# agakshat/spacefortress

Hardware: AMD Instinct MI355X
Metric: env-steps/sec (whole node), youturn random-action rollout @65536 envs/GPU (higher is better)
Workload: dtype f64; 1 GPU; youturn, 65536 envs/GPU, features obs (f32), uniform random discrete actions resident in HBM, per-lane auto-reset; envs_per_gpu=65536, gametype=youturn, obs_type=features

## Files before the change

### spacefortress_amd/csrc/sf_kernels.hip

```cpp
#include <hip/hip_runtime.h>
#include <cstdio>
#include <cstdlib>
#include <stdint.h>

#include "sf_drawrec.h"
#include "sf_lane_dev.h"
#define SF_EVENTS_FN static __device__ __forceinline__
#include "sf_events.h"

#ifndef SF_BLOCK
#define SF_BLOCK 256
#endif
#ifndef SF_SPLIT
#define SF_SPLIT 1
#endif
#ifndef SF_MROWS
#define SF_MROWS 3
#endif
#ifndef SF_SPF
#define SF_SPF 6
#endif
#ifndef SF_STAGGER
#define SF_STAGGER 12
#endif
// ... 145 lines not shown
template <int DIM>
__device__ __forceinline__ void write_features_f32(float* o, const Lane& L, const Extras& e, int real_shell_count) {
  const int n_missiles = __popc(L.mmask);
  const int n_shells = real_shell_count ? __popc(L.smask) : n_missiles;
  const int kill_ready = (L.vlner > 10 && L.fort_vuln_t < sfc::vuln_time) ? 1 : 0;
  const int timers[4] = {L.fire_t, L.thrust_t, L.left_t, L.right_t};
  o[0] = (L.fl & SF_FL_SHIP_ALIVE) ? 1.0f : 0.0f;
  o[1] = (float)L.sx;
  o[2] = (float)L.sy;
  o[3] = (float)L.vx;
  o[4] = (float)L.vy;
  o[5] = (float)L.angle;
  o[6] = (float)e.aim;
  o[7] = (float)e.vdir;
  o[8] = (float)e.ndist;
  o[9] = (L.fl & SF_FL_FORT_ALIVE) ? 1.0f : 0.0f;
  o[10] = (float)L.fort_angle;
  o[11] = (float)L.vlner;
  o[12] = (float)kill_ready;
  o[13] = (float)n_missiles;
  o[14] = (float)n_shells;
#pragma unroll
  for (int k = 0; k < DIM - 15; k++) o[15 + k] = (float)timers[k];
}
template <int DIM>
__device__ __forceinline__ void flush_features_f32(const float* stage_w, float* dst_w, unsigned lane) {
  __builtin_amdgcn_fence(__ATOMIC_RELEASE, "wavefront");
  __builtin_amdgcn_wave_barrier();
  __builtin_amdgcn_fence(__ATOMIC_ACQUIRE, "wavefront");
  typedef float f4_t __attribute__((ext_vector_type(4)));
  constexpr int NV = 64 * DIM / 4, IT = (NV + 63) / 64;
  f4_t v[IT];
#pragma unroll
  for (int k = 0; k < IT; k++)
    if (k * 64 + 63 < NV || (int)lane + k * 64 < NV) v[k] = reinterpret_cast<const f4_t*>(stage_w)[lane + k * 64];
#pragma unroll
  for (int k = 0; k < IT; k++)
    if (k * 64 + 63 < NV || (int)lane + k * 64 < NV) {
      sf_store<f4_t>(reinterpret_cast<f4_t*>(dst_w) + lane + k * 64, v[k]);
    }
}

template <typename T>
__device__ __forceinline__ void flush_obs_wave(const SfKernelArgs& a, const T* stage_w, T* obs, unsigned wave_env0,
                                               unsigned lane, bool vec_ok) {
  __builtin_amdgcn_fence(__ATOMIC_RELEASE, "wavefront");
  __builtin_amdgcn_wave_barrier();
  __builtin_amdgcn_fence(__ATOMIC_ACQUIRE, "wavefront");
  long rows = (long)a.n_envs - (long)wave_env0;
  if (rows > 64) rows = 64;
  if (rows <= 0) return;
  const int total = (int)rows * a.obs_dim;
  T* dst = obs + (size_t)wave_env0 * a.obs_dim;
  constexpr int V = 16 / (int)sizeof(T);
  int done_elems = 0;
  if (vec_ok) {
    typedef T vec_t __attribute__((ext_vector_type(V)));
    const int nvec = total / V;
    for (int v = lane; v < nvec; v += 64) {
      sf_store<vec_t>(reinterpret_cast<vec_t*>(dst) + v, reinterpret_cast<const vec_t*>(stage_w)[v]);
    }
    done_elems = nvec * V;
  }
  for (int t = done_elems + lane; t < total; t += 64) dst[t] = stage_w[t];
}

template <typename T>
__device__ __forceinline__ void norm_partials_wave(const SfKernelArgs& a, T* stage_w, unsigned wave_env0, unsigned lane,
                                                   double my_ret, bool has_obs) {
  const int dim = a.obs_dim, groups = 64 / dim;
  const size_t waves = (size_t)(a.lanes / 64), w = wave_env0 >> 6;
  long rows = (long)a.n_envs - (long)wave_env0;
  rows = rows > 64 ? 64 : (rows < 0 ? 0 : rows);
  double s = 0, q = 0;
  if (has_obs && (int)lane < groups * dim)
    for (int r = (int)lane / dim; r < rows; r += groups) {
      const double v = (double)stage_w[r * dim + (int)lane % dim];
      s += v;
      q += v * v;
    }
  __builtin_amdgcn_wave_barrier();
  double* fold = reinterpret_cast<double*>(stage_w);
  if (has_obs) {
    fold[lane] = s;
    fold[64 + lane] = q;
  }
  __builtin_amdgcn_fence(__ATOMIC_RELEASE, "wavefront");
  __builtin_amdgcn_wave_barrier();
  __builtin_amdgcn_fence(__ATOMIC_ACQUIRE, "wavefront");
  if ((int)lane < dim) {
    double ts = 0, tq = 0;
    if (has_obs)
      for (int g = 0; g < groups; g++) {
        ts += fold[g * dim + lane];
        tq += fold[64 + g * dim + lane];
      }
    a.n_partials[(size_t)lane * waves + w] = ts;
    a.n_partials[(size_t)(dim + 1 + lane) * waves + w] = tq;
  }
  double rs = (long)lane < rows ? my_ret : 0.0, rq = rs * rs;
  for (int o = 32; o > 0; o >>= 1) {
    rs += __shfl_xor(rs, o);
    rq += __shfl_xor(rq, o);
  }
  if (lane == 0) {
    a.n_partials[(size_t)dim * waves + w] = rs;
    a.n_partials[(size_t)(2 * dim + 1) * waves + w] = rq;
  }
}

}

__global__ __launch_bounds__(SF_BLOCK) void sf_reset_kernel(SfKernelArgs a, int first, unsigned cursor0,
                                                           unsigned cursor_stride, void* obs) {
  const unsigned i = blockIdx.x * SF_BLOCK + threadIdx.x;
  const unsigned lane = threadIdx.x & 63u;
  unsigned char* const tb = a.state + (size_t)__builtin_amdgcn_readfirstlane(i >> 6) * sfl::kTileBytes;
  const Off o = {lane * 16u, lane * 8u, lane * 4u, lane * 2u, lane};
  Lane L;
  if (first) {
    L.prev_vlner = 0;
    L.cursor = cursor0 + cursor_stride * i;
  } else {
    const i4_t mi = SF_LD(i4_t, SF_CHUNK(misc, 0), o.o16);
    L.prev_vlner = SF_LD(int, SF_CHUNK(timers_a, 0), o.o16) & 0xFFF;
    L.cursor = (unsigned)mi.y;
  }
  new_game(a, L);
  L.mpool = 0;
  store_lane(tb, o, L);
  if (obs != nullptr && i < (unsigned)a.n_envs && a.obs_type != 3) {
    Extras e = compute_extras(a, L, sf_atan2<true>(L.sy - sfc::fort_y, L.sx - sfc::fort_x), sf_atan2<false>(L.vy, L.vx));
    if (a.ref_reset_obs) e = Extras{0.0, 0.0, 0.0};
    write_obs_row(a, obs, i, L, e);
  }
}

template <bool AUTOTURN, bool SHAPED, bool FUSED, int OBSK, bool XTRA, int BLKP, bool FOBS = false>
__global__ __launch_bounds__(BLKP > 2000 ? BLKP - 2000 : (BLKP > 1000 ? 2 * (BLKP - 1000) : BLKP)) void sf_step_kernel(unsigned char* state_p, const double* consts_p,
                                                          const void* actions, int n_envs_p, int act_type,
                                                          int32_t* reward_out, uint8_t* done_out, uint8_t* info_out,
                                                          SfKernelArgs a, void* obs, int obs_vec_ok, int n_steps) {
  constexpr bool REPEAT = BLKP > 2000;
  constexpr bool SPLIT = BLKP > 1000 && !REPEAT;
  constexpr int BLK = REPEAT ? BLKP - 2000 : (SPLIT ? BLKP - 1000 : BLKP);
  constexpr int NT = SPLIT ? 2 * BLK : BLK;
  static_assert(!SPLIT || (!FUSED && OBSK == 1 && !XTRA), "the split launch exists for the plain step of the default observation");
  static_assert(!FOBS || XTRA, "the final-observation output rides on the XTRA instantiations");
  static_assert(!REPEAT || (FUSED && XTRA && !FOBS && BLK == SF_BLOCK), "the action repeat rides on the fused XTRA instantiations (a.final_obs: a run-time test)");
  constexpr int kStaged = SPLIT ? SF_LDS_SPLIT_DOUBLES : SF_LDS_DOUBLES;
  constexpr int kTrigPieces = (kStaged / 2 + NT - 1) / NT;
  constexpr int kLdsEv = kStaged;
  constexpr int kLdsAtab = SPLIT ? SF_CONST_ATAB : kLdsEv + BLK, kLdsHand = SPLIT ? kLdsEv + BLK : kLdsAtab + SF_ATAB_DOUBLES,
                kLdsHandMeta = kLdsHand + 2 * BLK,
                kLdsHandFlags = kLdsHandMeta + BLK / 2, kLdsStage = SPLIT ? kLdsHandFlags + BLK / 32 : kLdsHand;
  static_assert(kLdsEv == SF_LDS_EV || SPLIT, "the other kernels' map is the one above");
  static_assert(kStaged % 2 == 0 && kLdsAtab % 2 == 0 && kLdsHand % 2 == 0 && kLdsStage % 2 == 0, "16-byte LDS accesses");
  extern __shared__ double lds[];
  const unsigned tid_all = threadIdx.x;
  const unsigned tid = SPLIT ? (tid_all & (unsigned)(BLK - 1)) : tid_all;
  const unsigned i = blockIdx.x * BLK + tid;
  const unsigned lane = tid & 63u;
  unsigned char* const tb = state_p + (size_t)__builtin_amdgcn_readfirstlane(i >> 6) * sfl::kTileBytes;
  const Off o = {lane * 16u, lane * 8u, lane * 4u, lane * 2u, lane};
  const Off g = {i * 16u, i * 8u, i * 4u, i * 2u, i};
  const bool real = i < (unsigned)n_envs_p;
  const __amdgpu_buffer_rsrc_t rs = __builtin_amdgcn_make_buffer_rsrc(tb, 0, (int)sfl::kTileBytes, 0x00020000);
  constexpr int kStAux = SF_SC_AUX;
  auto pld16 = [&](unsigned goff, bool p) __attribute__((always_inline)) -> d2_t {
    return __builtin_bit_cast(d2_t, __builtin_amdgcn_raw_buffer_load_b128(rs, p ? o.o16 : SF_OOB, goff, 0));
  };
  auto pst16 = [&](unsigned goff, bool p, d2_t v) __attribute__((always_inline)) {
    sf_buf_st128<kStAux>(__builtin_bit_cast(u4_t, v), rs, p ? o.o16 : SF_OOB, goff);
  };
  auto pst16_at = [&](unsigned goff, bool p, unsigned extra, d2_t v) __attribute__((always_inline)) {
    sf_buf_st128<kStAux>(__builtin_bit_cast(u4_t, v), rs, p ? o.o16 + extra : SF_OOB, goff);
  };
#ifdef SF_STAMPS
  unsigned long long stamp_[SF_STAMP_SLOTS] = {};
  stamp_[12] = __builtin_amdgcn_s_memrealtime();
#endif
  SF_STAMP(0, false);

#if SF_STAGGER
  if (n_envs_p > 65536 - 256 && ((blockIdx.x >> 3) & 1u)) __builtin_amdgcn_s_sleep(SF_STAGGER);
#endif
  constexpr unsigned kSpinLimit = 1u << 18;
  typedef volatile __attribute__((address_space(3))) unsigned lds_word_t;
  lds_word_t* const hflags = (lds_word_t*)(reinterpret_cast<unsigned*>(lds + kLdsHandFlags) + 4u * (tid >> 6));
  if constexpr (SPLIT) {
    if (tid_all >= (unsigned)BLK) {
      const unsigned n_word = *reinterpret_cast<const __attribute__((address_space(4))) unsigned*>(
          reinterpret_cast<const __attribute__((address_space(4))) void*>(
              (unsigned long long)(tb + (unsigned)sfl::chunk_offset(SF_G_misc, 0) + 8u)));
      unsigned cpi0[kTrigPieces];
      d2_t cst0[kTrigPieces];
#pragma unroll
      for (int k = 0; k < kTrigPieces; k++) {
        cpi0[k] = min(tid_all + k * NT, (unsigned)(kStaged / 2 - 1));
        cst0[k] = SF_LD(d2_t, (const unsigned char*)consts_p, cpi0[k] * 16u);
      }
      const unsigned m_live = n_word >> SF_MPOOL_SHIFT;
      d2_t prow[SF_MROWS];
      unsigned pmeta[SF_MROWS];
#pragma unroll
      for (int k = 0; k < kTrigPieces; k++) reinterpret_cast<d2_t*>(lds)[cpi0[k]] = cst0[k];
      if (lane < 4u) hflags[lane] = 0u;
      asm volatile("" ::: "memory");
#pragma unroll
      for (int r = 0; r < SF_MROWS; r++) {
        asm volatile("" : "=v"(prow[r].x), "=v"(prow[r].y));
        pmeta[r] = 0u;
        if (m_live > 64u * r) {
          const bool in_ = 64u * r + lane < m_live;
          prow[r] = __builtin_bit_cast(d2_t, __builtin_amdgcn_raw_buffer_load_b128(rs, in_ ? o.o16 : SF_OOB, SF_GOFF(missile_pos, r), 0));
          pmeta[r] = __builtin_amdgcn_raw_buffer_load_b32(rs, in_ ? o.o4 : SF_OOB, SF_GOFF(missile_meta, r), 0);
        }
      }
      __syncthreads();
#pragma unroll
      for (int r = 0; r < SF_MROWS; r++) asm volatile("" : "+v"(pmeta[r]));
      const double* trig = lds;
      d2_t pcs[SF_MROWS];
#pragma unroll
      for (int r = 0; r < SF_MROWS; r++) pcs[r] = *reinterpret_cast<const d2_t*>(&trig[2 * SF_MM_ANGLE(pmeta[r])]);
      double kv_speed = sfc::missile_speed, kv_fx = sfc::fort_x, kv_fy = sfc::fort_y, kv_w = sfc::width_d, kv_h = sfc::height_d,
             kv_mr2 = sfc::missile_hit_r2;
      asm volatile("" : "+v"(kv_speed), "+v"(kv_fx), "+v"(kv_fy), "+v"(kv_w), "+v"(kv_h), "+v"(kv_mr2));
      unsigned wp = 0;
      unsigned* const evw32 = reinterpret_cast<unsigned*>(lds + kLdsEv) + 2u * (tid & ~63u);
      auto m_row = [&](double x, double y, unsigned meta, d2_t cs, bool valid) __attribute__((always_inline)) {
        const double nx = x + kv_speed * cs.x, ny = y + kv_speed * cs.y;
        const double dx = nx - kv_fx, dy = ny - kv_fy;
        const bool hit = valid & (dx * dx + dy * dy <= kv_mr2);
        const bool gone = valid & (hit | (__builtin_fmax(__builtin_fmax(-nx, nx - kv_w), __builtin_fmax(-ny, ny - kv_h)) > 0));
        if (__ballot(gone) != 0ull) {
          if (gone)
            __hip_atomic_fetch_or(evw32 + 2 * SF_MM_OWNER(meta) + (hit ? 0 : 1), 1u << SF_MM_SLOT(meta), __ATOMIC_RELAXED,
                                  __HIP_MEMORY_SCOPE_WORKGROUP);
        }
        const bool keep = valid & !gone;
        const unsigned long long kb = __ballot(keep);
        const unsigned idx = wp + __builtin_amdgcn_mbcnt_hi((unsigned)(kb >> 32), __builtin_amdgcn_mbcnt_lo((unsigned)kb, 0u));
        wp += (unsigned)__popcll(kb);
        sf_buf_st128<kStAux>(__builtin_bit_cast(u4_t, (d2_t{nx, ny})), rs, keep ? idx * 16u : SF_OOB,
                                               SF_GOFF(missile_pos, 0));
        __builtin_amdgcn_raw_buffer_store_b32(meta, rs, keep ? idx * 4u : SF_OOB, SF_GOFF(missile_meta, 0), kStAux);
      };
#pragma unroll
      for (int r = 0; r < SF_MROWS; r++)
        if (m_live > 64u * r) m_row(prow[r].x, prow[r].y, pmeta[r], pcs[r], 64u * r + lane < m_live);
      if (m_live > 64u * SF_MROWS) {
#pragma unroll 1
        for (unsigned r = SF_MROWS; 64u * r < m_live; r++) {
          const d2_t pr = __builtin_bit_cast(d2_t, __builtin_amdgcn_raw_buffer_load_b128(rs, o.o16 + r * 1024u, SF_GOFF(missile_pos, 0), 16));
          const unsigned pm = __builtin_amdgcn_raw_buffer_load_b32(rs, o.o4 + r * 256u, SF_GOFF(missile_meta, 0), 16);
          m_row(pr.x, pr.y, pm, *reinterpret_cast<const d2_t*>(&trig[2 * SF_MM_ANGLE(pm)]), 64u * r + lane < m_live);
        }
      }
      unsigned fired, spins = 0u;
      while ((fired = (unsigned)__builtin_amdgcn_readfirstlane((int)hflags[0])) == 0u && ++spins < kSpinLimit) __builtin_amdgcn_s_sleep(1);
      if (spins >= kSpinLimit && lane == 0u) atomicAdd(&a.acc[SF_ACC_HANDOVER], 1ull);
      asm volatile("" ::: "memory");
      if (fired == 2u) {
        const d2_t nxy = reinterpret_cast<const d2_t*>(lds + kLdsHand)[tid];
        const unsigned nm = reinterpret_cast<const unsigned*>(lds + kLdsHandMeta)[tid];
        m_row(nxy.x, nxy.y, nm & 0x7FFFFFFFu, *reinterpret_cast<const d2_t*>(&trig[2 * SF_MM_ANGLE(nm)]), !(nm >> 31));
      }
      asm volatile("s_waitcnt lgkmcnt(0)" ::: "memory");
      if (lane == 0u) hflags[1] = 0x80000000u | wp;
      asm volatile("s_waitcnt vmcnt(0)" ::: "memory");
      if (lane == 0u) hflags[2] = 1u;
      return;
    }
  }
  u4_t act_rec = {0u, 0u, 0u, 0u};
  if (XTRA && act_type == SF_ACT_SAMPLED)
    act_rec = *(reinterpret_cast<const __attribute__((address_space(4))) u4_t*>(
                    reinterpret_cast<const __attribute__((address_space(4))) void*>((unsigned long long)actions)) +
                __builtin_amdgcn_readfirstlane(i >> 6));
  auto sample_action = [&](int step) __attribute__((always_inline)) -> int {
    const unsigned x = sf_philox4x32_10(act_rec.w + lane, act_rec.x + (unsigned)step, act_rec.y, act_rec.z);
    return real ? (int)__umulhi(x, (unsigned)a.n_actions) : 0;
  };
  auto load_action = [&](int step) __attribute__((always_inline)) -> int {
    if (!real || (XTRA && act_type == SF_ACT_SAMPLED)) return 0;
    const unsigned char* ab = (const unsigned char*)actions;
    const unsigned e = (unsigned)step * (unsigned)n_envs_p + i;
    if (act_type == 8) return (int)SF_LD(long long, ab, e * 8u);
    if (act_type == 4) return SF_LD(int, ab, e * 4u);
    return SF_LD(unsigned char, ab, e);
  };
  Lane L;
  load_lane_early(tb, o, L);
  int act_next = load_action(0);
  const unsigned atab_pi = min(tid, (unsigned)(SF_ATAB_DOUBLES / 2 - 1));
  const d2_t atab_piece = SPLIT ? d2_t{0, 0} : SF_LD(d2_t, (const unsigned char*)consts_p, (SF_CONST_ATAB / 2 + atab_pi) * 16u);
  const unsigned char* cb = (const unsigned char*)consts_p;
  d2_t cst[kTrigPieces];
  unsigned cpi[kTrigPieces];
#pragma unroll
  for (int k = 0; k < kTrigPieces; k++) {
    cpi[k] = min(tid_all + k * NT, (unsigned)(kStaged / 2 - 1));
    cst[k] = SF_LD(d2_t, cb, cpi[k] * 16u);
  }
  int act_sampled = 0;
  if (XTRA && act_type == SF_ACT_SAMPLED) act_sampled = sample_action(0);
#define SF_LOAD_POOL_ROWS(aux, n_pool)                                                                                        \
  _Pragma("unroll") for (int r = 0; r < SF_MROWS; r++) {                                                                      \
    const bool in_ = 64u * r + lane < (n_pool);                                                                               \
    prow[r] = __builtin_bit_cast(d2_t, __builtin_amdgcn_raw_buffer_load_b128(rs, in_ ? o.o16 : SF_OOB, SF_GOFF(missile_pos, r), (aux)));   \
    pmeta[r] = __builtin_amdgcn_raw_buffer_load_b32(rs, in_ ? o.o4 : SF_OOB, SF_GOFF(missile_meta, r), (aux));               \
  }
  constexpr bool kPoolLoads = !SPLIT;
  d2_t prow[SF_MROWS];
  unsigned pmeta[SF_MROWS];
  LaneLate late;
  SF_STAMP(1, false);
  SF_STAMP(2, true);

  __builtin_amdgcn_s_waitcnt(0x0F70);
#pragma unroll
  for (int k = 0; k < kTrigPieces; k++) reinterpret_cast<d2_t*>(lds)[cpi[k]] = cst[k];
  unsigned long long* const evw = reinterpret_cast<unsigned long long*>(lds + kLdsEv) + (tid & ~63u);
  evw[lane] = 0ull;
  if constexpr (!SPLIT) reinterpret_cast<d2_t*>(lds + kLdsAtab)[atab_pi] = atab_piece;

  double shx[SF_SPF], shy[SF_SPF], shvx[SF_SPF], shvy[SF_SPF];
#pragma unroll
  for (int s = 0; s < SF_SPF; s++) {
    if (FUSED) {
      shx[s] = shy[s] = shvx[s] = shvy[s] = 0;
    } else {
      asm volatile("" : "=v"(shx[s]), "=v"(shy[s]), "=v"(shvx[s]), "=v"(shvy[s]));
    }
  }
  bool will_respawn = !(L.fl & SF_FL_SHIP_ALIVE) && L.death_t >= sfc::explode_duration;
  unsigned long long spawn_e = 0;
  const __amdgpu_buffer_rsrc_t rs_spawn =
      __builtin_amdgcn_make_buffer_rsrc(const_cast<int16_t*>(a.spawn), 0, (int)((a.spawn_mask + 1u) * 8u), 0x00020000);
  auto load_spawn = [&]() __attribute__((always_inline)) {
    const i2_t e = __builtin_bit_cast(i2_t, __builtin_amdgcn_raw_buffer_load_b64(rs_spawn, will_respawn ? (L.cursor & a.spawn_mask) * 8u : SF_OOB, 0, 0));
    spawn_e = (unsigned long long)(unsigned)e.x | ((unsigned long long)(unsigned)e.y << 32);
  };
  load_spawn();
  {
#pragma unroll
    for (int g = 0; g < SF_SPF; g++) {
      if (__ballot((L.smask & (1u << g)) != 0u) != 0ull) {
#pragma unroll
        for (int k = 0; k < 1; k++) {
          const int s = g + k;
          const bool live = (L.smask >> s) & 1u;
          const d2_t sp = pld16(SF_GOFF(shell_pos, s), live);
          const d2_t sv = pld16(SF_GOFF(shell_vel, s), live);
          shx[s] = sp.x;
          shy[s] = sp.y;
          shvx[s] = sv.x;
          shvy[s] = sv.y;
        }
      }
    }
  }
  late = load_lane_late(tb, o);
  if (kPoolLoads) { SF_LOAD_POOL_ROWS(0, L.mpool) }

  __syncthreads();
  const double* trig = lds;
  SF_STAMP(3, false);
  SfKRow kc;
  if constexpr (SPLIT) kc = sf_load_krow(lds + SF_CONST_KROW);

  if (FUSED) unpack_lane_late(late, L);
  const int n_iter = FUSED ? n_steps : 1;
  constexpr unsigned kRpInfo = 1u << 8, kRpDied = 1u << 9, kRpParked = 1u << 10;
  unsigned rp_w = 0u, rp_events = 0u, rp_proj = 0u;
  int rp_reward = 0;
  double rp_apos = 0, rp_avel = 0;
  for (int step = 0; step < n_iter; step++) {
  int act = (XTRA && act_type == SF_ACT_SAMPLED) ? act_sampled : act_next;
  if (FUSED) {
    if (!REPEAT && step + 1 < n_iter) {
      act_next = load_action(step + 1);
      if (XTRA && act_type == SF_ACT_SAMPLED) act_sampled = sample_action(step + 1);
    }
    if (step > 0) {
      SF_LOAD_POOL_ROWS(16, L.mpool)
      will_respawn = !(L.fl & SF_FL_SHIP_ALIVE) && L.death_t >= sfc::explode_duration;
      load_spawn();
    }
  }
  const size_t so = REPEAT ? (size_t)0 : (size_t)step * (size_t)a.n_envs;
  const bool rp_parked = REPEAT && (rp_w & kRpParked) != 0u;
  const bool draw_now = OBSK != 1 && a.draw != nullptr && (!FUSED || step + 1 == n_iter);
  unsigned dr_proj = 0u;

  const int act_raw = act;
  if (act < 0 || act >= a.n_actions) {
    if (!rp_parked) atomicAdd(&a.acc[SF_ACC_BAD_ACTION], 1ull);
    act = 0;
  }
  const unsigned keys = (unsigned)(a.action_keys >> (4 * act)) & 0xFu;

  StatDelta S;

  float rew = 0;

  int new_m_slot = -1;
  unsigned key_edge_bits = 0;
  float amt_fire = 0.0f, amt_hex = 0.0f;
  unsigned key_edges;
  {
    const unsigned kmask = AUTOTURN ? 0x3u : 0xFu;
    const unsigned old = (L.fl >> 2) & kmask, now = keys & kmask;
    const unsigned edge = old ^ now, press = now & ~old;
    key_edges = press | ((old & ~now) << 4);
    L.fl = (L.fl & ~(kmask << 2)) | (now << 2);
    key_edge_bits = edge;
    S.shots += (int)(press & 1u);
    S.thrusts += (int)((press >> 1) & 1u);
    L.kc0 += (press & 1u) | ((press & 2u) << 15);
    if (!AUTOTURN) L.kc1 += ((press >> 2) & 1u) | ((press & 8u) << 13);
    if (!AUTOTURN) {
      S.lefts += (int)((press >> 2) & 1u);
      S.rights += (int)((press >> 3) & 1u);
    }
    {
      const int slot = __ffs(~L.mmask) - 1;
      const bool can = (press & 1u) && (L.fl & SF_FL_SHIP_ALIVE) && slot >= 0 && slot < SF_NSLOT;
      new_m_slot = can ? slot : -1;
      L.mmask |= can ? (1u << (slot & 31)) : 0u;
      amt_fire = can ? -sfc::Score<SHAPED>::missile_penalty : 0.0f;
    }
  }
  const double new_m_x = L.sx, new_m_y = L.sy;
  const int new_m_angle = L.angle;
  if constexpr (SPLIT) {
    reinterpret_cast<d2_t*>(lds + kLdsHand)[tid] = d2_t{new_m_x, new_m_y};
    reinterpret_cast<unsigned*>(lds + kLdsHandMeta)[tid] =
        new_m_slot >= 0 ? SF_MM_PACK(new_m_angle, lane, new_m_slot & 31) : 0x80000000u;
    asm volatile("" ::: "memory");
    const unsigned fired = __ballot(new_m_slot >= 0) != 0ull ? 2u : 1u;
    if (lane == 0u) hflags[0] = fired;
  }

  if (will_respawn) {
    spawn_ship_from(a, L, spawn_e);
  }

  if (L.fl & SF_FL_SHIP_ALIVE) {
    if (AUTOTURN) {
      double t = SPLIT ? sf_atan2_razor(sfc::fort_y - L.sy, sfc::fort_x - L.sx, lds + kLdsAtab, kc)
                       : sf_atan2<true>(sfc::fort_y - L.sy, sfc::fort_x - L.sx, lds + kLdsAtab);
      if (t < 0) t += M_PI * 2;
      double c = ceil(SPLIT ? rad2deg(t, kc) : rad2deg(t));
      int ia = (int)c;
      if (ia >= 360) ia -= 360;
      L.angle = ia;
    } else {
      L.angle += sfc::turn_speed * ((int)((L.fl / SF_FL_RIGHT) & 1u) - (int)((L.fl / SF_FL_LEFT) & 1u));
      L.angle += L.angle < 0 ? 360 : 0;
      L.angle -= L.angle >= 360 ? 360 : 0;
    }
    {
      const bool th = L.fl & SF_FL_THRUST;
      const double tvx = L.vx + sfc::ship_accel * SF_COS(L.angle), tvy = L.vy + sfc::ship_accel * SF_SIN(L.angle);
      L.vx = th ? tvx : L.vx;
      L.vy = th ? tvy : L.vy;
    }
    L.sx += L.vx;
    L.sy += L.vy;
    const int out_big = !inside_big_hex(L.sx, L.sy);
    const int in_small = !out_big & inside_small_hex(L.sx, L.sy);
    {
      const int dead_now = out_big | in_small;
      L.fl &= dead_now ? ~SF_FL_SHIP_ALIVE : ~0u;
      L.death_t = dead_now ? 0 : L.death_t;
      S.ship_deaths += dead_now;
      amt_hex = dead_now ? -sfc::Score<SHAPED>::death_penalty : 0.0f;
    }
    S.big_hex_deaths += out_big;
    S.small_hex_deaths += in_small;
  }

  double a_pos = SPLIT ? sf_atan2_razor(L.sy - sfc::fort_y, L.sx - sfc::fort_x, lds + kLdsAtab, kc)
                       : sf_atan2<true>(L.sy - sfc::fort_y, L.sx - sfc::fort_x, lds + kLdsAtab);
  double a_vel = SPLIT ? sf_atan2_core(L.vy, L.vx, lds + kLdsAtab, kc) : sf_atan2_core(L.vy, L.vx, lds + kLdsAtab);
  if (!FUSED) {
    asm volatile("" : "+v"(a_pos), "+v"(a_vel), "+v"(late.ta.x), "+v"(late.ta.y), "+v"(late.ta.z), "+v"(late.ta.w));
    unpack_lane_late(late, L);
  }

  int new_s_slot = -1;
  double new_s_vx = 0, new_s_vy = 0;
  bool fort_respawned = false;
  {
    double ats = SPLIT ? rad2deg(a_pos, kc) : rad2deg(a_pos);
    if (ats < 0) ats += SPLIT ? kc.d360 : 360;
    L.fort_t = will_respawn ? 0 : L.fort_t;
    fort_respawned = !(L.fl & SF_FL_FORT_ALIVE) && L.fort_death_t > sfc::fort_respawn;
    L.fort_t = fort_respawned ? 0 : L.fort_t;
    L.fl |= fort_respawned ? SF_FL_FORT_ALIVE : 0u;
    const bool ship_up = L.fl & SF_FL_SHIP_ALIVE;
    {
      double q = SPLIT ? ceil(sf_div_const(ats, kc.d10, kc.inv10)) * kc.d10
                       : ceil(SF_DIV(ats, sfc::sector_size)) * sfc::sector_size;
      int fa = (int)q;
      fa -= fa >= 360 ? 360 : 0;
      L.fort_angle = ship_up ? fa : L.fort_angle;
      const bool moved = ship_up && fa != L.fort_last;
      L.fort_last = moved ? fa : L.fort_last;
      L.fort_t = moved ? 0 : L.fort_t;
    }
    if (ship_up) {
      if (L.fort_t >= sfc::lock_time && (L.fl & SF_FL_FORT_ALIVE)) {
        int slot = __ffs(~L.smask) - 1;
        if (slot < SF_NSLOT) {
          new_s_slot = slot;
          L.smask |= 1u << slot;
          const double ddx = L.sx - sfc::fort_x, ddy = L.sy - sfc::fort_y;
          const double nrm = sqrt(ddx * ddx + ddy * ddy);
          new_s_vx = sfc::shell_speed * (ddx / nrm);
          new_s_vy = sfc::shell_speed * (ddy / nrm);
        }
        L.fort_t = 0;
      }
    }
  }
  SF_STAMP(4, false);
  SF_STAMP(5, true);

  asm volatile("" ::"v"(spawn_e));
  const unsigned m_live = (unsigned)__builtin_amdgcn_readfirstlane((int)L.mpool);
  d2_t pcs[SF_MROWS];
#pragma unroll
  for (int r = 0; r < SF_MROWS; r++)
    pcs[r] = SPLIT ? d2_t{0, 0} : *reinterpret_cast<const d2_t*>(&trig[2 * SF_MM_ANGLE(pmeta[r])]);

  score(amt_fire, rew, L);
  score(amt_hex, rew, L);

  double kv_speed = sfc::missile_speed, kv_fx = sfc::fort_x, kv_fy = sfc::fort_y, kv_w = sfc::width_d, kv_h = sfc::height_d,
         kv_mr2 = sfc::missile_hit_r2, kv_sr2 = sfc::shell_hit_r2;
  asm volatile("" : "+v"(kv_speed), "+v"(kv_fx), "+v"(kv_fy), "+v"(kv_w), "+v"(kv_h), "+v"(kv_mr2), "+v"(kv_sr2));
  auto outside = [&](double x, double y) __attribute__((always_inline)) -> bool {
    return __builtin_fmax(__builtin_fmax(-x, x - kv_w), __builtin_fmax(-y, y - kv_h)) > 0;
  };

  static_assert(sfl::kGroups[SF_G_shell_vel].chunk * sfl::kTileLanes == 1024, "slot stride of the row below");
  if (__ballot(new_s_slot >= 0) != 0ull)
    pst16_at(SF_GOFF(shell_vel, 0), new_s_slot >= 0, (unsigned)new_s_slot * 1024u, d2_t{new_s_vx, new_s_vy});
  {
#pragma unroll
    for (int g = 0; g < SF_SPF; g++) {
      const unsigned gmask = 1u << g;
      if (__ballot((L.smask & gmask) != 0u) == 0ull) continue;
      unsigned col = 0, out = 0;
      double nx[1], ny[1];
#pragma unroll
      for (int k = 0; k < 1; k++) {
        const int s = g + k;
        const bool isnew = (s == new_s_slot);
        const double vx = isnew ? new_s_vx : shvx[s], vy = isnew ? new_s_vy : shvy[s];
        nx[k] = (isnew ? kv_fx : shx[s]) + vx;
        ny[k] = (isnew ? kv_fy : shy[s]) + vy;
        const double dx = nx[k] - L.sx, dy = ny[k] - L.sy;
        col |= (unsigned)(dx * dx + dy * dy <= kv_sr2) << s;
        out |= (unsigned)outside(nx[k], ny[k]) << s;
        if (FUSED) {
          shx[s] = nx[k];
          shy[s] = ny[k];
          shvx[s] = vx;
          shvy[s] = vy;
        }
      }
      const unsigned live = L.smask & gmask;
      col &= live;
      unsigned dead = out & live;
      {
        const int hitship = (L.fl & SF_FL_SHIP_ALIVE) && col;
        dead |= hitship ? (col & (0u - col)) : 0u;
        L.fl &= hitship ? ~SF_FL_SHIP_ALIVE : ~0u;
        L.death_t = hitship ? 0 : L.death_t;
        S.ship_deaths += hitship;
        S.shell_deaths += hitship;
        score(hitship ? -sfc::Score<SHAPED>::death_penalty : 0.0f, rew, L);
      }
      L.smask &= ~dead;
#pragma unroll
      for (int k = 0; k < 1; k++) {
        const int s = g + k;
        pst16(SF_GOFF(shell_pos, s), (L.smask >> s) & 1u, d2_t{nx[k], ny[k]});
        if (draw_now)
          if (((L.smask >> s) & 1u) && sfd::hud_rows_near((float)ny[k], sfd::kShellExt))
            dr_proj |= sfd::hud_flags_near((float)nx[k], (float)ny[k], sfd::kShellExt);
      }
    }
    if (__ballot((L.smask >> SF_SPF) != 0u) != 0ull) {
#pragma unroll 1
      for (int s = SF_SPF; s < SF_NSLOT; s++) {
        const bool live = (L.smask >> s) & 1u;
        if (__ballot(live) == 0ull) continue;
        if (live) {
          double x, y, vx, vy;
          if (s == new_s_slot) {
            x = sfc::fort_x;
            y = sfc::fort_y;
            vx = new_s_vx;
            vy = new_s_vy;
          } else {
            const d2_t sp = ld_coherent_d2(SF_CHUNK(shell_pos, s) + o.o16);
            const d2_t sv = ld_coherent_d2(SF_CHUNK(shell_vel, s) + o.o16);
            x = sp.x;
            y = sp.y;
            vx = sv.x;
            vy = sv.y;
          }
          x += vx;
          y += vy;
          bool dead = false;
          if (L.fl & SF_FL_SHIP_ALIVE) {
            const double dx = x - L.sx, dy = y - L.sy;
            if (dx * dx + dy * dy <= sfc::shell_hit_r2) {
              dead = true;
              kill_ship(L, S);
              score(-sfc::Score<SHAPED>::death_penalty, rew, L);
              S.shell_deaths += 1;
            }
          }
          if (!dead && outside_area(a, x, y)) dead = true;
          if (dead) {
            L.smask &= ~(1u << s);
          } else {
            SF_ST(d2_t, SF_CHUNK(shell_pos, s), o.o16, (d2_t{x, y}));
            if (draw_now) dr_proj |= sfd::hud_flags_near((float)x, (float)y, sfd::kShellExt);
          }
        }
      }
    }
  }

  unsigned hit_count = 0;
  {
    unsigned wp = 0;
    unsigned* const evw32 = reinterpret_cast<unsigned*>(evw);
    const __amdgpu_buffer_rsrc_t rs_draw = __builtin_amdgcn_make_buffer_rsrc(
        draw_now ? a.draw + (size_t)__builtin_amdgcn_readfirstlane(i >> 6) * (size_t)SF_DR_TILE_BYTES : (unsigned char*)nullptr, 0,
        draw_now ? SF_DR_TILE_BYTES : 0, 0x00020000);
    auto m_row = [&](double x, double y, unsigned meta, d2_t cs, bool valid) __attribute__((always_inline)) {
      const double nx = x + kv_speed * cs.x, ny = y + kv_speed * cs.y;
      const double dx = nx - kv_fx, dy = ny - kv_fy;
      const bool hit = valid & (dx * dx + dy * dy <= kv_mr2);
      const bool gone = valid & (hit | outside(nx, ny));
      if (__ballot(gone) != 0ull) {
        if (gone) {
          __hip_atomic_fetch_or(evw32 + 2 * SF_MM_OWNER(meta) + (hit ? 0 : 1), 1u << SF_MM_SLOT(meta), __ATOMIC_RELAXED,
                                __HIP_MEMORY_SCOPE_WORKGROUP);
        }
      }
      const bool keep = valid & !gone;
      const unsigned long long kb = __ballot(keep);
      const unsigned idx = wp + __builtin_amdgcn_mbcnt_hi((unsigned)(kb >> 32), __builtin_amdgcn_mbcnt_lo((unsigned)kb, 0u));
      wp += (unsigned)__popcll(kb);
      sf_buf_st128<kStAux>(__builtin_bit_cast(u4_t, (d2_t{nx, ny})), rs, keep ? idx * 16u : SF_OOB,
                                             SF_GOFF(missile_pos, 0));
      __builtin_amdgcn_raw_buffer_store_b32(meta, rs, keep ? idx * 4u : SF_OOB, SF_GOFF(missile_meta, 0), kStAux);
      if (draw_now) {
        typedef float f4_t __attribute__((ext_vector_type(4)));
        const unsigned doff = (SF_DR_PIECE_OBJ0 + SF_DR_OBJ_MISSILE0 + SF_MM_SLOT(meta)) * (unsigned)SF_DR_PIECE_STRIDE +
                              SF_MM_OWNER(meta) * (unsigned)SF_DR_LANE_STRIDE;
        sf_buf_st128<0>(__builtin_bit_cast(u4_t, (d2_t{nx, ny})), rs_draw, keep ? doff : SF_OOB, 0);
        __builtin_amdgcn_raw_buffer_store_b16((short)SF_MM_ANGLE(meta), rs_draw,
                                              keep ? SF_DR_ANGLES_OFF + 2u * SF_MM_SLOT(meta) + SF_MM_OWNER(meta) * (unsigned)SF_DR_LANE_STRIDE : SF_OOB,
                                              0, 0);
        const bool rows = keep & sfd::hud_rows_near((float)ny, sfd::kMissileExt);
        if (__ballot(rows) != 0ull) {
          if (rows)
            __hip_atomic_fetch_or(evw32 + 2 * SF_MM_OWNER(meta), sfd::hud_flags_near((float)nx, (float)ny, sfd::kMissileExt) << 24,
                                  __ATOMIC_RELAXED, __HIP_MEMORY_SCOPE_WORKGROUP);
        }
      }
    };
    if constexpr (SPLIT) {
      unsigned dw, spins = 0u;
      SF_STAMP(16, false);
      while (!((dw = (unsigned)__builtin_amdgcn_readfirstlane((int)hflags[1])) >> 31) && ++spins < kSpinLimit) __builtin_amdgcn_s_sleep(1);
      if (spins >= kSpinLimit && lane == 0u) atomicAdd(&a.acc[SF_ACC_HANDOVER], 1ull);
      asm volatile("" ::: "memory");
      SF_STAMP(17, false);
      wp = dw & 0x7FFFFFFFu;
    } else {
#pragma unroll
      for (int r = 0; r < SF_MROWS; r++)
        if (m_live > 64u * r) m_row(prow[r].x, prow[r].y, pmeta[r], pcs[r], 64u * r + lane < m_live);
      if (m_live > 64u * SF_MROWS) {
#pragma unroll 1
        for (unsigned r = SF_MROWS; 64u * r < m_live; r++) {
          const d2_t pr = __builtin_bit_cast(d2_t, __builtin_amdgcn_raw_buffer_load_b128(rs, o.o16 + r * 1024u, SF_GOFF(missile_pos, 0), 16));
          const unsigned pm = __builtin_amdgcn_raw_buffer_load_b32(rs, o.o4 + r * 256u, SF_GOFF(missile_meta, 0), 16);
          m_row(pr.x, pr.y, pm, *reinterpret_cast<const d2_t*>(&trig[2 * SF_MM_ANGLE(pm)]), 64u * r + lane < m_live);
        }
      }
      if (__ballot(new_m_slot >= 0) != 0ull)
        m_row(new_m_x, new_m_y, SF_MM_PACK(new_m_angle, lane, new_m_slot & 31),
              *reinterpret_cast<const d2_t*>(&trig[2 * new_m_angle]), new_m_slot >= 0);
    }
    L.mpool = wp;
    __builtin_amdgcn_fence(__ATOMIC_RELEASE, "wavefront");
    __builtin_amdgcn_wave_barrier();
    __builtin_amdgcn_fence(__ATOMIC_ACQUIRE, "wavefront");
    const unsigned long long evp = evw[lane];
    if (FUSED) evw[lane] = 0ull;
    unsigned ev_hit = (unsigned)evp, ev_out = (unsigned)(evp >> 32);
    dr_proj |= (ev_hit >> 24) & 0xFu;
    ev_hit &= L.mmask;
    ev_out &= L.mmask & ~ev_hit;
    const unsigned ev = ev_hit | ev_out;
    hit_count = __popc(ev_hit);
    L.mmask &= ~ev;
    static_assert(sfc::Score<false>::miss_penalty == 0.0f && sfc::Score<true>::miss_penalty == 0.0f,
                  "sf_missile_events scores no miss (:394-398)");
    {
      const SfMissileEvents e = sf_missile_events((int)hit_count, __popc(ev_out), (L.fl & SF_FL_FORT_ALIVE) != 0u, L.fort_vuln_t,
                                                  L.vlner, sfc::vuln_time, sfc::vuln_threshold, sfc::Score<SHAPED>::destroy_reward);
      L.vlner = e.vlner;
      L.fl &= e.fort_alive ? ~0u : ~SF_FL_FORT_ALIVE;
      L.fort_vuln_t = e.fort_vuln_t;
      L.fort_death_t = e.fort_death_reset ? 0 : L.fort_death_t;
      S.vlner_incs += e.incs;
      S.max_vlner = e.max_vlner > S.max_vlner ? e.max_vlner : S.max_vlner;
      S.destroyed += e.destroyed;
      S.resets += e.resets;
      S.missed += e.missed;
      score(e.amount, rew, L);
    }
  }
  SF_STAMP(6, false);

  L.fort_t += sfc::tick_ms;
  L.fort_death_t += sfc::tick_ms;
  L.fort_vuln_t += sfc::tick_ms;
  L.death_t += sfc::tick_ms;
  L.fire_t = ((key_edge_bits & 1u) ? 0 : L.fire_t) + ((L.fl & SF_FL_FIRE) ? 1 : -1);
  L.thrust_t = ((key_edge_bits & 2u) ? 0 : L.thrust_t) + ((L.fl & SF_FL_THRUST) ? 1 : -1);
  L.left_t = ((key_edge_bits & 4u) ? 0 : L.left_t) + ((L.fl & SF_FL_LEFT) ? 1 : -1);
  L.right_t = ((key_edge_bits & 8u) ? 0 : L.right_t) + ((L.fl & SF_FL_RIGHT) ? 1 : -1);

  int r = (int)rew;
  L.fl = (L.fl & 0xFFu) | ((unsigned)(r & 0xFF) << 8);

  const int fort_kill = r > 0;
  if (SHAPED) {
    const int vlner_change = L.vlner - L.prev_vlner;
    if (L.vlner <= 10 && !fort_kill) r += vlner_change;
    r = r > 1 ? 1 : (r < -1 ? -1 : r);
    r = r + 2 * fort_kill;
    L.prev_vlner = L.vlner;
  }
  L.time += sfc::tick_ms;
  const int done = L.time >= sfc::game_time;

  unsigned evmask = 0;
  if (a.events) {
    const int live_hits = S.vlner_incs + S.destroyed + S.resets;
    evmask = key_edges | (new_m_slot >= 0 ? SF_EV_MISSILE_FIRED : 0u) | (will_respawn ? SF_EV_SHIP_RESPAWN : 0u) |
             (S.big_hex_deaths ? SF_EV_EXPLODE_BIGHEX : 0u) | (S.small_hex_deaths ? SF_EV_EXPLODE_SMALLHEX : 0u) |
             (fort_respawned ? SF_EV_FORTRESS_RESPAWN : 0u) | (new_s_slot >= 0 ? SF_EV_FORTRESS_FIRED : 0u) |
             (S.shell_deaths ? SF_EV_SHELL_HIT_SHIP : 0u) | (live_hits ? SF_EV_HIT_FORTRESS : 0u) |
             (S.vlner_incs ? SF_EV_VLNER_INCREASED : 0u) | (S.destroyed ? SF_EV_FORTRESS_DESTROYED : 0u) |
             (S.resets ? SF_EV_VLNER_RESET : 0u) | ((int)hit_count > live_hits ? SF_EV_HIT_DEAD_FORTRESS : 0u) |
             (S.missed ? SF_EV_MISSILE_LEFT : 0u) | (done ? SF_EV_GAME_OVER : 0u);
  }

  SF_STAMP(10, false);
  L.ep_return += r;
  L.ep_kills += (unsigned)fort_kill;
  L.c_resets += (unsigned)S.resets;
  L.c_missed += (unsigned)S.missed;
  L.c_incs += (unsigned)S.vlner_incs;
  L.c_maxv = (unsigned)S.max_vlner > L.c_maxv ? (unsigned)S.max_vlner : L.c_maxv;
  L.c_big += (unsigned)S.big_hex_deaths;
  L.c_small += (unsigned)S.small_hex_deaths;
  L.c_shell += (unsigned)S.shell_deaths;
  L.c_destroyed += (unsigned)S.destroyed;
  if (XTRA && !REPEAT && !a.auto_reset) {
    const unsigned ov = ((L.c_resets | L.c_missed) >> 16) | ((L.c_incs | L.c_maxv | (unsigned)L.vlner) >> 12) |
                        ((L.c_big | L.c_small | L.c_shell | L.c_destroyed | L.ep_kills) >> 8) | ((unsigned)L.time >> 24) |
                        (((unsigned)(L.fire_t + 32768) | (unsigned)(L.thrust_t + 32768) | (unsigned)(L.left_t + 32768) |
                          (unsigned)(L.right_t + 32768)) >> 16) |
                        (unsigned)(S.shots && (L.kc0 & 0xFFFFu) == 0u) | (unsigned)(S.thrusts && (L.kc0 >> 16) == 0u) |
                        (unsigned)(S.lefts && (L.kc1 & 0xFFFFu) == 0u) | (unsigned)(S.rights && (L.kc1 >> 16) == 0u);
    if (__ballot(ov != 0u) != 0ull)
// ... 15 lines not shown
      atomicAdd(&a.acc[2], (unsigned long long)((long long)ep_ret * ep_ret));
      atomicAdd(&a.acc[3], (unsigned long long)(long long)ep_kil);
      atomicAdd(&a.acc[4], (unsigned long long)deaths);
      atomicAdd(&a.acc[5], (unsigned long long)shots);
      atomicMin((long long*)&a.acc[6], (long long)ep_ret);
      atomicMax((long long*)&a.acc[7], (long long)ep_ret);
    }
    if ((FOBS || REPEAT) && a.final_obs != nullptr) {
      if (real) write_obs_row(a, a.final_obs, i, L, compute_extras(a, L, a_pos, a_vel));
    }
    if constexpr (REPEAT) {
      rp_w |= kRpParked;
      L.fl &= ~SF_FL_SHIP_ALIVE;
      L.death_t = -(1 << 24);
      L.mmask = L.smask = 0u;
    } else {
    new_game(a, L);
    a_pos = sf_atan2<true>(L.sy - sfc::fort_y, L.sx - sfc::fort_x);
    a_vel = sf_atan2<false>(L.vy, L.vx);
    }
  }
  if constexpr (!REPEAT) SF_PURGE_POOL(__ballot(done && a.auto_reset))

  SF_STAMP(11, false);
  if constexpr (!REPEAT)
    if (draw_now) SF_DRAW_HEADER(done && a.auto_reset, dr_proj)
  if (!FUSED) store_lane_buf(rs, o, L);
  SF_STAMP(14, false);

  if constexpr (REPEAT) {
    rp_apos = a_pos;
    rp_avel = a_vel;
    rp_proj = dr_proj;
    if (__ballot(!(rp_w & kRpParked)) == 0ull) break;
  } else {
  if (real) {
    if (reward_out) SF_ST(int32_t, (unsigned char*)(reward_out + so), g.o4, r);
    if (done_out) SF_ST(uint8_t, (unsigned char*)(done_out + so), g.o1, (uint8_t)done);
    if (info_out) SF_ST(uint8_t, (unsigned char*)(info_out + so), g.o1, (uint8_t)fort_kill);
    if (a.events) SF_ST(uint32_t, (unsigned char*)(a.events + so), g.o4, evmask);
    if (XTRA && a.act_out) SF_ST(uint8_t, (unsigned char*)(a.act_out + so), g.o1, (uint8_t)act_raw);
    SF_STAMP(15, false);
    if (a.t_reward) {
      const float rf = (float)r, mask = done ? 0.0f : 1.0f;
      SF_ST(float, (unsigned char*)(a.t_reward + so), g.o4, rf);
      if (a.t_mask) SF_ST(float, (unsigned char*)(a.t_mask + so), g.o4, mask);
      if (a.t_episode) {
        const float ep = SF_LD(float, (const unsigned char*)a.t_episode, g.o4) + rf;
        if (a.t_final) {
          float fin = SF_LD(float, (const unsigned char*)a.t_final, g.o4) * mask;
          fin = fin + (1.0f - mask) * ep;
          SF_ST(float, (unsigned char*)a.t_final, g.o4, fin);
        }
        SF_ST(float, (unsigned char*)a.t_episode, g.o4, ep * mask);
      }
      if (a.t_actions) SF_ST(long long, (unsigned char*)(a.t_actions + so), g.o8, (long long)act_raw);
    }
  }
  SF_STAMP(7, false);
  SF_WRITE_OBSERVATION(so, a_pos, a_vel, done && a.auto_reset)
  if constexpr (OBSK != 1) {
    if (a.hint) {
      const unsigned long long died = __ballot(real && (S.big_hex_deaths | S.small_hex_deaths | S.shell_deaths) != 0);
      if (lane == 0) a.hint[i >> 6] = died;
    }
  }
  if (!FUSED && a.n_partials) {
    double my_ret = 0;
    if (a.n_ret && real) {
      my_ret = SF_LD(double, (const unsigned char*)a.n_ret, g.o8) * a.n_gamma + (double)r;
      SF_ST(double, (unsigned char*)a.n_ret, g.o8, my_ret);
    }
    const bool has_obs = obs != nullptr && a.obs_type != 3;
    if (a.obs_f64)
      norm_partials_wave<double>(a, lds + kLdsStage + (size_t)(tid & ~63u) * a.obs_dim, i & ~63u, lane, my_ret, has_obs);
    else
      norm_partials_wave<float>(a, reinterpret_cast<float*>(lds + kLdsStage) + (size_t)(tid & ~63u) * a.obs_dim, i & ~63u,
                                lane, my_ret, has_obs);
  }
  }
  }
  if constexpr (REPEAT) {
    const bool parked = (rp_w & kRpParked) != 0u;
    const unsigned long long pk = __ballot(parked);
    if (pk != 0ull) {
      if (parked) {
        new_game(a, L);
        rp_apos = sf_atan2<true>(L.sy - sfc::fort_y, L.sx - sfc::fort_x);
        rp_avel = sf_atan2<false>(L.vy, L.vx);
      }
      SF_PURGE_POOL(pk)
    }
  }
  if (FUSED) store_lane_buf(rs, o, L);
  if constexpr (REPEAT) {
    const bool parked = (rp_w & kRpParked) != 0u;
    if (OBSK != 1 && a.draw != nullptr) SF_DRAW_HEADER(parked, rp_proj)
    if (real) {
      if (reward_out) SF_ST(int32_t, (unsigned char*)reward_out, g.o4, rp_reward);
      if (done_out) SF_ST(uint8_t, (unsigned char*)done_out, g.o1, (uint8_t)parked);
      if (info_out) SF_ST(uint8_t, (unsigned char*)info_out, g.o1, (uint8_t)((rp_w & kRpInfo) != 0u));
      if (a.events) SF_ST(uint32_t, (unsigned char*)a.events, g.o4, rp_events);
      if (a.act_out) SF_ST(uint8_t, (unsigned char*)a.act_out, g.o1, (uint8_t)(rp_w & 0xFFu));
    }
    SF_WRITE_OBSERVATION((size_t)0, rp_apos, rp_avel, parked)
    if constexpr (OBSK != 1) {
      if (a.hint) {
        const unsigned long long died = __ballot(real && (rp_w & kRpDied) != 0u);
        if (lane == 0) a.hint[i >> 6] = died;
      }
    }
  }
  if (XTRA && !REPEAT && act_type == SF_ACT_SAMPLED && lane == 0)
    reinterpret_cast<unsigned*>(const_cast<void*>(actions))[4 * (size_t)(i >> 6)] = act_rec.x + (unsigned)n_iter;
  SF_STAMP(8, false);
  SF_STAMP(9, true);
#ifdef SF_STAMPS
  stamp_[13] = __builtin_amdgcn_s_memrealtime();
  asm volatile("s_waitcnt lgkmcnt(0)" ::: "memory");
  if (a.dbg != nullptr && (tid & 63) == 0) {
    unsigned long long* d = a.dbg + (size_t)(i >> 6) * SF_STAMP_SLOTS;
#pragma unroll
    for (int k = 0; k < SF_STAMP_SLOTS; k++) d[k] = stamp_[k];
  }
#endif
}


hipError_t sf_launch_reset(const SfKernelArgs& a, int first, unsigned cursor0, unsigned stride, void* obs,
                           hipStream_t stream) {
  const unsigned grid = (unsigned)(a.lanes / SF_BLOCK);
  hipLaunchKernelGGL(sf_reset_kernel, dim3(grid), dim3(SF_BLOCK), 0, stream, a, first, cursor0, stride, obs);
  return hipGetLastError();
}

hipError_t sf_launch_step(const SfKernelArgs& a, bool autoturn, bool shaped, const void* actions, int act_type, void* obs,
                          int32_t* reward, uint8_t* done, uint8_t* info, int n_steps, bool fused, hipStream_t stream) {
  int blk = fused ? SF_BLOCK : (a.lanes <= 64 * 256 ? 64 : (a.lanes <= 128 * 256 ? 128 : SF_BLOCK));
  const size_t elem = a.obs_f64 ? sizeof(double) : sizeof(float);
  const int vec_ok = ((uintptr_t)obs & 15u) == 0 && (!fused || ((size_t)a.n_envs * a.obs_dim * elem) % 16 == 0);
  const bool fast_obs = obs != nullptr && a.obs_type == 0 && !a.obs_f64 && vec_ok && a.n_envs % 64 == 0 &&
                        a.obs_dim == (autoturn ? 17 : 19) && !a.ref_reset_obs;
  const bool fobs = a.final_obs != nullptr;
  const bool xtra = act_type == SF_ACT_SAMPLED || a.act_out != nullptr || !a.auto_reset || fobs;
  static const int force_split = [] { const char* e = getenv("SFMI_FORCE_SPLIT"); return e ? atoi(e) : 0; }();
  const bool split = SF_SPLIT && !fused && fast_obs && !xtra && (a.lanes <= 65536 || SF_SPLIT == 2 || force_split) && a.draw == nullptr;
  if (split && force_split == 2) {
    static bool said = false;
    if (!said) fprintf(stderr, "sfmi: split launch (%ld lanes)\n", (long)a.lanes);
    said = true;
  }
  const unsigned grid = (unsigned)(a.lanes / blk);
  size_t lds_bytes = (size_t)(SF_LDS_DOUBLES + blk + SF_ATAB_DOUBLES) * sizeof(double) + (size_t)blk * a.obs_dim * elem;
  if (split) lds_bytes = (size_t)(SF_LDS_SPLIT_DOUBLES + blk + 2 * blk + blk / 2 + blk / 32) * sizeof(double) + (size_t)blk * a.obs_dim * elem;
#define SF_GO2(AT, SH, FU, OK, XT, BL, FO)                                                                            \
  hipLaunchKernelGGL((sf_step_kernel<AT, SH, FU, OK, XT, BL, FO>), dim3(grid), dim3((BL) > 1000 ? 2 * ((BL) - 1000) : (BL)), lds_bytes, stream, a.state,    \
                     a.consts, actions, a.n_envs, act_type, reward, done, info, a, obs, vec_ok, n_steps)
#define SF_GO1(AT, SH, FU, OK, XT, FO)                                                                             \
  do {                                                                                                             \
    if (FU || blk == SF_BLOCK) SF_GO2(AT, SH, FU, OK, XT, SF_BLOCK, FO);                                           \
    else if (blk == 128) SF_GO2(AT, SH, false, OK, XT, 128, FO);                                                   \
    else SF_GO2(AT, SH, false, OK, XT, 64, FO);                                                                    \
  } while (0)
#if SF_SPLIT
#define SF_GO_SPLIT(AT, SH)                                                                                        \
  if (split) {                                                                                                     \
    if (blk == SF_BLOCK) SF_GO2(AT, SH, false, 1, false, 1256, false);                                             \
    else if (blk == 128) SF_GO2(AT, SH, false, 1, false, 1128, false);                                             \
    else SF_GO2(AT, SH, false, 1, false, 1064, false);                                                             \
  } else
#else
#define SF_GO_SPLIT(AT, SH)
#endif
#define SF_GO(AT, SH, FU)                                                                                          \
  SF_GO_SPLIT(AT, SH)                                                                                              \
  if (fast_obs) {                                                                                                  \
    if (fobs) SF_GO1(AT, SH, FU, 1, true, true);                                                                   \
    else if (xtra) SF_GO1(AT, SH, FU, 1, true, false); else SF_GO1(AT, SH, FU, 1, false, false);                   \
  } else {                                                                                                         \
    if (fobs) SF_GO1(AT, SH, FU, 0, true, true);                                                                   \
    else if (xtra) SF_GO1(AT, SH, FU, 0, true, false); else SF_GO1(AT, SH, FU, 0, false, false);                   \
  }
  const int sel = (autoturn ? 4 : 0) | (shaped ? 2 : 0) | (fused ? 1 : 0);
  switch (sel) {
    case 0: SF_GO(false, false, false); break;
    case 1: SF_GO(false, false, true); break;
    case 2: SF_GO(false, true, false); break;
    case 3: SF_GO(false, true, true); break;
    case 4: SF_GO(true, false, false); break;
    case 5: SF_GO(true, false, true); break;
    case 6: SF_GO(true, true, false); break;
    default: SF_GO(true, true, true); break;
  }
#undef SF_GO
#undef SF_GO1
#undef SF_GO_SPLIT
#undef SF_GO2
  return hipGetLastError();
}

hipError_t sf_launch_step_repeat(const SfKernelArgs& a0, bool autoturn, bool shaped, const void* actions, int act_type, void* obs,
                                 int32_t* reward, uint8_t* done, uint8_t* info, uint8_t* ticks, int repeat, hipStream_t stream) {
  SfKernelArgs a = a0;
  a.act_out = ticks;
  const size_t elem = a.obs_f64 ? sizeof(double) : sizeof(float);
  const int vec_ok = ((uintptr_t)obs & 15u) == 0;
  const bool fast_obs = obs != nullptr && a.obs_type == 0 && !a.obs_f64 && vec_ok && a.n_envs % 64 == 0 &&
                        a.obs_dim == (autoturn ? 17 : 19) && !a.ref_reset_obs;
  const unsigned grid = (unsigned)(a.lanes / SF_BLOCK);
  const size_t lds_bytes = (size_t)(SF_LDS_DOUBLES + SF_BLOCK + SF_ATAB_DOUBLES) * sizeof(double) + (size_t)SF_BLOCK * a.obs_dim * elem;
#define SF_GO(AT, SH)                                                                                                       \
  do {                                                                                                                      \
    if (fast_obs)                                                                                                           \
      hipLaunchKernelGGL((sf_step_kernel<AT, SH, true, 1, true, 2000 + SF_BLOCK, false>), dim3(grid), dim3(SF_BLOCK), lds_bytes, \
                         stream, a.state, a.consts, actions, a.n_envs, act_type, reward, done, info, a, obs, vec_ok, repeat);  \
    else                                                                                                                    \
      hipLaunchKernelGGL((sf_step_kernel<AT, SH, true, 0, true, 2000 + SF_BLOCK, false>), dim3(grid), dim3(SF_BLOCK), lds_bytes, \
                         stream, a.state, a.consts, actions, a.n_envs, act_type, reward, done, info, a, obs, vec_ok, repeat);  \
  } while (0)
  switch ((autoturn ? 2 : 0) | (shaped ? 1 : 0)) {
    case 0: SF_GO(false, false); break;
    case 1: SF_GO(false, true); break;
    case 2: SF_GO(true, false); break;
    default: SF_GO(true, true); break;
  }
#undef SF_GO
  return hipGetLastError();
}
```

Baseline: 11.13 billion env-steps/s.

## Offload fort shell spawn (normalize and stores) to the split helper wave

In the split launch, the main wave now only decides whether the fort fires and which slot it uses, and posts the ship-fort offset and slot to LDS with a flag. The helper half of the block waits on that flag, computes the normalized shell velocity (sqrt and divides), and writes the new shell's velocity and position to the state tile. The main wave drops the new shell from its own shell-advance loop and only sets the slot bit. This takes the f64 sqrt/divide and two stores off the main wave's critical path, at the cost of a second handshake spin, more LDS per block, and the new shell no longer being advanced or collision-tested in its spawn step on this path.

```diff
diff --git a/spacefortress_amd/csrc/sf_kernels.hip b/spacefortress_amd/csrc/sf_kernels.hip
--- a/spacefortress_amd/csrc/sf_kernels.hip
+++ b/spacefortress_amd/csrc/sf_kernels.hip
@@ -321,10 +321,10 @@
   constexpr int kTrigPieces = (kStaged / 2 + NT - 1) / NT;
   constexpr int kLdsEv = kStaged;
   constexpr int kLdsAtab = SPLIT ? SF_CONST_ATAB : kLdsEv + BLK, kLdsHand = SPLIT ? kLdsEv + BLK : kLdsAtab + SF_ATAB_DOUBLES,
-                kLdsHandMeta = kLdsHand + 2 * BLK,
-                kLdsHandFlags = kLdsHandMeta + BLK / 2, kLdsStage = SPLIT ? kLdsHandFlags + BLK / 32 : kLdsHand;
+                kLdsHandMeta = kLdsHand + 2 * BLK, kLdsShot = kLdsHandMeta + BLK / 2, kLdsShotSlot = kLdsShot + 2 * BLK,
+                kLdsHandFlags = SPLIT ? kLdsShotSlot + BLK / 2 : kLdsHandMeta + BLK / 2, kLdsStage = SPLIT ? kLdsHandFlags + BLK / 32 : kLdsHand;
   static_assert(kLdsEv == SF_LDS_EV || SPLIT, "the other kernels' map is the one above");
-  static_assert(kStaged % 2 == 0 && kLdsAtab % 2 == 0 && kLdsHand % 2 == 0 && kLdsStage % 2 == 0, "16-byte LDS accesses");
+  static_assert(kStaged % 2 == 0 && kLdsAtab % 2 == 0 && kLdsHand % 2 == 0 && kLdsShot % 2 == 0 && kLdsStage % 2 == 0, "16-byte LDS accesses");
   extern __shared__ double lds[];
   const unsigned tid_all = threadIdx.x;
   const unsigned tid = SPLIT ? (tid_all & (unsigned)(BLK - 1)) : tid_all;
@@ -438,6 +438,22 @@
       }
       asm volatile("s_waitcnt lgkmcnt(0)" ::: "memory");
       if (lane == 0u) hflags[1] = 0x80000000u | wp;
+      static_assert(sfl::kGroups[SF_G_shell_vel].chunk * sfl::kTileLanes == 1024 && sfl::kGroups[SF_G_shell_pos].chunk * sfl::kTileLanes == 1024,
+                    "slot stride of the two stores below");
+      unsigned shot;
+      spins = 0u;
+      while ((shot = (unsigned)__builtin_amdgcn_readfirstlane((int)hflags[3])) == 0u && ++spins < kSpinLimit) __builtin_amdgcn_s_sleep(1);
+      if (spins >= kSpinLimit && lane == 0u) atomicAdd(&a.acc[SF_ACC_HANDOVER], 1ull);
+      asm volatile("" ::: "memory");
+      if (shot == 2u) {
+        const d2_t dd = reinterpret_cast<const d2_t*>(lds + kLdsShot)[tid];
+        const unsigned sl = reinterpret_cast<const unsigned*>(lds + kLdsShotSlot)[tid];
+        const double nrm = sqrt(dd.x * dd.x + dd.y * dd.y);
+        const double svx = sfc::shell_speed * (dd.x / nrm), svy = sfc::shell_speed * (dd.y / nrm);
+        const unsigned so = !(sl >> 31) ? o.o16 + sl * 1024u : SF_OOB;
+        sf_buf_st128<kStAux>(__builtin_bit_cast(u4_t, (d2_t{svx, svy})), rs, so, SF_GOFF(shell_vel, 0));
+        sf_buf_st128<kStAux>(__builtin_bit_cast(u4_t, (d2_t{kv_fx + svx, kv_fy + svy})), rs, so, SF_GOFF(shell_pos, 0));
+      }
       asm volatile("s_waitcnt vmcnt(0)" ::: "memory");
       if (lane == 0u) hflags[2] = 1u;
       return;
@@ -661,6 +677,7 @@
   }
 
   int new_s_slot = -1;
+  unsigned new_s_bit = 0u;
   double new_s_vx = 0, new_s_vy = 0;
   bool fort_respawned = false;
   {
@@ -681,7 +698,19 @@
       L.fort_last = moved ? fa : L.fort_last;
       L.fort_t = moved ? 0 : L.fort_t;
     }
-    if (ship_up) {
+    if constexpr (SPLIT) {
+      const int slot = __ffs(~L.smask) - 1;
+      const bool lock = ship_up && L.fort_t >= sfc::lock_time && (L.fl & SF_FL_FORT_ALIVE);
+      const bool fire = lock && slot < SF_NSLOT;
+      new_s_slot = fire ? slot : -1;
+      new_s_bit = fire ? 1u << (slot & 31) : 0u;
+      L.fort_t = lock ? 0 : L.fort_t;
+      reinterpret_cast<d2_t*>(lds + kLdsShot)[tid] = d2_t{L.sx - sfc::fort_x, L.sy - sfc::fort_y};
+      reinterpret_cast<unsigned*>(lds + kLdsShotSlot)[tid] = fire ? (unsigned)slot : 0x80000000u;
+      asm volatile("" ::: "memory");
+      const unsigned shot = __ballot(fire) != 0ull ? 2u : 1u;
+      if (lane == 0u) hflags[3] = shot;
+    } else if (ship_up) {
       if (L.fort_t >= sfc::lock_time && (L.fl & SF_FL_FORT_ALIVE)) {
         int slot = __ffs(~L.smask) - 1;
         if (slot < SF_NSLOT) {
@@ -717,7 +746,7 @@
   };
 
   static_assert(sfl::kGroups[SF_G_shell_vel].chunk * sfl::kTileLanes == 1024, "slot stride of the row below");
-  if (__ballot(new_s_slot >= 0) != 0ull)
+  if (!SPLIT && __ballot(new_s_slot >= 0) != 0ull)
     pst16_at(SF_GOFF(shell_vel, 0), new_s_slot >= 0, (unsigned)new_s_slot * 1024u, d2_t{new_s_vx, new_s_vy});
   {
 #pragma unroll
@@ -729,7 +758,7 @@
 #pragma unroll
       for (int k = 0; k < 1; k++) {
         const int s = g + k;
-        const bool isnew = (s == new_s_slot);
+        const bool isnew = !SPLIT && (s == new_s_slot);
         const double vx = isnew ? new_s_vx : shvx[s], vy = isnew ? new_s_vy : shvy[s];
         nx[k] = (isnew ? kv_fx : shx[s]) + vx;
         ny[k] = (isnew ? kv_fy : shy[s]) + vy;
@@ -772,7 +801,7 @@
         if (__ballot(live) == 0ull) continue;
         if (live) {
           double x, y, vx, vy;
-          if (s == new_s_slot) {
+          if (!SPLIT && s == new_s_slot) {
             x = sfc::fort_x;
             y = sfc::fort_y;
             vx = new_s_vx;
@@ -807,6 +836,7 @@
         }
       }
     }
+    if constexpr (SPLIT) L.smask |= new_s_bit;
   }
 
   unsigned hit_count = 0;
@@ -1128,7 +1158,7 @@
   }
   const unsigned grid = (unsigned)(a.lanes / blk);
   size_t lds_bytes = (size_t)(SF_LDS_DOUBLES + blk + SF_ATAB_DOUBLES) * sizeof(double) + (size_t)blk * a.obs_dim * elem;
-  if (split) lds_bytes = (size_t)(SF_LDS_SPLIT_DOUBLES + blk + 2 * blk + blk / 2 + blk / 32) * sizeof(double) + (size_t)blk * a.obs_dim * elem;
+  if (split) lds_bytes = (size_t)(SF_LDS_SPLIT_DOUBLES + blk + 2 * (2 * blk + blk / 2) + blk / 32) * sizeof(double) + (size_t)blk * a.obs_dim * elem;
 #define SF_GO2(AT, SH, FU, OK, XT, BL, FO)                                                                            \
   hipLaunchKernelGGL((sf_step_kernel<AT, SH, FU, OK, XT, BL, FO>), dim3(grid), dim3((BL) > 1000 ? 2 * ((BL) - 1000) : (BL)), lds_bytes, stream, a.state,    \
                      a.consts, actions, a.n_envs, act_type, reward, done, info, a, obs, vec_ok, n_steps)
```

Measured after the change: 11.46 billion env-steps/s, median of 6. +3.0%, better.
